# maxipalay/ekf-slam

Measured on AMD Instinct MI355X. Metric: EKF correction steps/sec at N landmarks; pose RMSE vs reference, higher is better.
Workload: dtype f32; 1 GPU; n1024_fp32; n_landmarks=1024, state_dim=2051, filters_per_gpu=1, filters_total=1, markers_per_message=16, association=known, seeds=20240317 + global filter index, survey_messages=640, landmarks_initialised_min=1024, landmarks_initialised_target=1024, inputs=hbm, parallelism=independent filters x1 ranks

## Files before the change

### ekf-slam_amd/csrc/ekf_api.cpp

```cpp
#include <algorithm>
#include <cstdlib>
#include <new>
#include <vector>

#include "ekf_ctx.hpp"
#include "geom.hpp"

using namespace ekfslam;

namespace {

bool valid(ekf_ctx* h, int f) { return h && f >= 0 && f < h->F; }

int load_and_plan(ekf_ctx* h, int assoc_mode, int m_max, const int* counts, const int* ids,
                  const int* actions, const double* rel_xy, const double* odom) {
  Planner& p = h->plan;
  if (int rc = p.load_batch(assoc_mode, m_max, counts, ids, actions, rel_xy, odom)) return rc;
  if (assoc_mode)
    p.unknown(0, h->F, true, true, 0, p.largest(h->F), p.absent(), assoc_route(h));
  else
    p.known(0, h->F, true, p.absent());
  return EKF_OK;
}

// ... 47 lines not shown
  h->ld = (h->n + per_line - 1) / per_line * per_line;
  h->ldk = (h->n + 63) / 64 * 64;
  h->sig_stride = static_cast<size_t>(h->n) * h->ld;
  h->x_stride = static_cast<size_t>((h->n + 15) / 16 * 16);
  h->km_stride = static_cast<size_t>(kMaxKW) * h->ldk;
  h->held.assign(h->F, 0);
  auto fail = [&](int rc) {
    ekf_destroy(h);
    return rc;
  };
  if (hipSetDevice(cfg.device) != hipSuccess) return fail(EKF_E_HIP);
  const char* serial_env = std::getenv("EKF_SERIAL");
  if (serial_env) h->serial = std::atoi(serial_env) != 0;
  if (const char* e = std::getenv("EKF_ASSOC_MSG")) h->assoc_msg = std::atoi(e) != 0;
  {
    const char* e = std::getenv("EKF_RESIDENT");
    h->resident = cfg.dtype == EKF_F64 && h->n <= kResidentMaxN && !(e && std::atoi(e) == 0);
  }
  if (create_streams(h) != EKF_OK ||
      hipEventCreateWithFlags(&h->ev_chain, hipEventDisableTiming) != hipSuccess ||
      hipEventCreateWithFlags(&h->ev_join, hipEventDisableTiming) != hipSuccess ||
      hipEventCreateWithFlags(&h->ev_sig[0], hipEventDisableTiming) != hipSuccess ||
      hipEventCreateWithFlags(&h->ev_sig[1], hipEventDisableTiming) != hipSuccess)
    return fail(EKF_E_HIP);
  if (!serial_env && !h->devsync && h->F > kCuSplitMaxFilters) h->serial = true;
  h->am_route = am_route(h, false);
  h->am_route_j = am_route(h, true);
  if (hipHostMalloc(reinterpret_cast<void**>(&h->fatal_h), 64,
                    hipHostMallocMapped | hipHostMallocCoherent) != hipSuccess)
    return fail(EKF_E_NOMEM);
  *h->fatal_h = 0;
  if (hipHostGetDevicePointer(reinterpret_cast<void**>(&h->fatal_d), h->fatal_h, 0) != hipSuccess)
    return fail(EKF_E_HIP);
  const size_t sig_bytes = h->sig_stride * h->F * h->w;
  for (int p = 0; p < 2; ++p) {
    if (hipMalloc(&h->sig[p], sig_bytes) != hipSuccess) return fail(EKF_E_NOMEM);
    if (hipMalloc(&h->x[p], h->x_stride * h->F * sizeof(double)) != hipSuccess)
      return fail(EKF_E_NOMEM);
  }
  const size_t km_bytes = h->km_stride * h->F * h->w;
  if (hipMalloc(&h->kcat, km_bytes) != hipSuccess) return fail(EKF_E_NOMEM);
  if (hipMalloc(&h->mcat, km_bytes) != hipSuccess) return fail(EKF_E_NOMEM);
  if (hipMalloc(&h->ctl, sizeof(FilterCtl) * h->F) != hipSuccess) return fail(EKF_E_NOMEM);
  if (hipMalloc(&h->rec, 2 * sizeof(ChunkRec) * h->F) != hipSuccess) return fail(EKF_E_NOMEM);
  const char* stage_env = std::getenv("EKF_STAGE");
  const size_t stage_bytes =
      2 * h->F * by_dtype(h, [](auto tag) { return sizeof(StageRec<decltype(tag)>); });
  const bool stage_on = stage_env ? std::atoi(stage_env) != 0
                                  : (h->devsync || h->F <= kCuSplitMaxFilters);
  if (stage_on) {
    if (hipMalloc(&h->stage, stage_bytes) != hipSuccess) return fail(EKF_E_NOMEM);
    if (hipMemset(h->stage, 0, stage_bytes) != hipSuccess) return fail(EKF_E_HIP);
  }
  h->plan.init(h->F, cfg.n_landmarks, h->resident, stage_on);
  const size_t sync_bytes = sizeof(unsigned) * (kSyncChain + static_cast<size_t>(h->F));
  if (hipMalloc(&h->sync, sync_bytes) != hipSuccess) return fail(EKF_E_NOMEM);
  if (hipMemset(h->sync, 0, sync_bytes) != hipSuccess) return fail(EKF_E_HIP);
  h->ddesc_cap = std::max(kDescInit, static_cast<size_t>(h->F) * 4);
  if (hipMalloc(&h->ddesc, sizeof(MsgDesc) * h->ddesc_cap) != hipSuccess) return fail(EKF_E_NOMEM);
  for (int i = 0; i < kRing; ++i)
    if (hipEventCreateWithFlags(&h->ring[i].ev, hipEventDisableTiming) != hipSuccess)
      return fail(EKF_E_HIP);
  if (int rc = reserve_upload(h, h->ddesc_cap)) return fail(rc);
  for (int p = 0; p < 2; ++p) {
    if (hipMemsetAsync(h->sig[p], 0, sig_bytes, h->stream) != hipSuccess) return fail(EKF_E_HIP);
    if (hipMemsetAsync(h->x[p], 0, h->x_stride * h->F * sizeof(double), h->stream) != hipSuccess)
      return fail(EKF_E_HIP);
  }
  if (hipMemsetAsync(h->rec, 0, 2 * sizeof(ChunkRec) * h->F, h->stream) != hipSuccess)
    return fail(EKF_E_HIP);
  if (hipMemsetAsync(h->kcat, 0, km_bytes, h->stream) != hipSuccess ||
      hipMemsetAsync(h->mcat, 0, km_bytes, h->stream) != hipSuccess ||
      hipMemsetAsync(h->ctl, 0, sizeof(FilterCtl) * h->F, h->stream) != hipSuccess)
    return fail(EKF_E_HIP);
  if (init_diag(h, h->sig[0], h->F) || hipStreamSynchronize(h->stream) != hipSuccess)
    return fail(EKF_E_HIP);
  *out = h;
  return EKF_OK;
}

int ekf_destroy(ekf_t h) {
  if (!h) return EKF_E_ARG;
  hipSetDevice(h->cfg.device);
  if (h->bulk) hipStreamSynchronize(h->bulk);
  if (h->stream) hipStreamSynchronize(h->stream);
  for (int p = 0; p < 2; ++p) {
    if (h->sig[p]) hipFree(h->sig[p]);
    if (h->x[p]) hipFree(h->x[p]);
  }
  if (h->kcat) hipFree(h->kcat);
  if (h->mcat) hipFree(h->mcat);
  if (h->ctl) hipFree(h->ctl);
  if (h->rec) hipFree(h->rec);
  if (h->stage) hipFree(h->stage);
  if (h->ddesc) hipFree(h->ddesc);
  for (PlanState* p : h->dstate)
    if (p) hipFree(p);
  if (h->hstate) hipHostFree(h->hstate);
  if (h->odom_d) hipFree(h->odom_d);
  if (h->odom_h) hipHostFree(h->odom_h);
  if (h->ev_odom) hipEventDestroy(h->ev_odom);
  if (h->fatal_h) hipHostFree(h->fatal_h);
  if (h->am.hist) hipFree(h->am.hist);
  if (h->am.cur) hipFree(h->am.cur);
  if (h->am.gran) hipFree(h->am.gran);
  for (int i = 0; i < kRing; ++i) {
// ... 392 lines not shown
```

### ekf-slam_amd/csrc/ekf_chain.hip

```cpp
#include <hip/hip_ext.h>
#include <hip/hip_runtime.h>

#include <cstdint>
#include <type_traits>

#include "ekf_device.hpp"
#include "ekf_launch.hpp"
#include "ekf_math.hpp"
#include "geom.hpp"

namespace ekfslam {

#include "ekf_diag.hpp"
#ifdef EKF_DIAG_STAMPS
__device__ unsigned long long g_stamps[4 * 512];
__device__ double g_blocks[64][kMaxU][kMaxU + 1];
__device__ double g_blockx[64][kMaxU];
}
extern "C" int ekfslam_diag_read_stamps(unsigned long long* out, int n) {
  using ekfslam::g_stamps;
  return hipMemcpyFromSymbol(out, HIP_SYMBOL(g_stamps), sizeof(unsigned long long) * (n < 2048 ? n : 2048)) == hipSuccess ? 0 : -5;
}
extern "C" int ekfslam_diag_read_blocks(double* blocks, double* xs) {
  using namespace ekfslam;
// ... 6 lines not shown
#include "ekf_sync.hpp"

template <bool J>
struct ChainSharedT {
  static constexpr int ZC = J ? kZJ : kZC;
  static constexpr int JM = J ? kMaxJoseph : 1;
  int u[kMaxU];
  int skip[kMaxChunk];
  double alphaU[kMaxU];
  double row0raw[kMaxU];
  double col0raw[kMaxU];
  double xU[1][kMaxU];
  RebuildImage<double> im;
  double Cz[kMaxChunk][4];
  double Dy[kMaxChunk][4];
  double KU[kMaxChunk][kMaxU][2];
  double MU[kMaxChunk][kMaxU][2];
  double Z[kMaxU][ZC + 1];
  double Y[kZC][kMaxU + 1];
  double Zx[kMaxU];
  double nu[kMaxChunk][2];
  double Hs[kMaxChunk][2][5];
  double Sis[kMaxChunk][4];
  double VU[JM][kMaxU][2];
  double Ss[JM][4];
  double Cv[JM][4];
  double Dv[JM][4];
  struct {
    int u[kMaxU];
    int nu, m, first, joseph;
    double a1, a2, s00;
    double xU[kMaxU], Zx[kMaxU];
    double Z[kMaxU + 1][ZC + 1];
    double Y[kZC][kMaxU + 1];
    double K[kMaxU][ZC + 1];
    double M[kZC][kMaxU + 1];
    double r0U[kMaxU], c0U[kMaxU], r0P[kMaxU], c0P[kMaxU];
    double xg[kMaxU];
  } pv;
  double junk[4][64];
  double junk2[64][2];
  double pose[3];
  double xpose[3];
  double npose[3], na1, na2;
  int npose_ci;
  double tmo[3];
  double a1, a2, s00;
  int nu_cnt;
  unsigned status;
  int pub;
  int pdone;
  int any_init;
  int zdone;
};

__device__ __forceinline__ void lds_publish(int* flag, int v) {
  __atomic_signal_fence(__ATOMIC_SEQ_CST);
  __hip_atomic_store(flag, v, __ATOMIC_RELAXED, __HIP_MEMORY_SCOPE_WORKGROUP);
}
__device__ __forceinline__ void lds_wait_ge(const int* flag, int v) {
  while (__builtin_amdgcn_readfirstlane(
             __hip_atomic_load(flag, __ATOMIC_ACQUIRE, __HIP_MEMORY_SCOPE_WORKGROUP)) < v)
    __builtin_amdgcn_s_sleep(1);
}

template <bool J>
using LdsChain = __attribute__((address_space(3))) ChainSharedT<J>;
typedef __attribute__((address_space(3))) const MsgDesc LdsDesc;
typedef __attribute__((address_space(3))) double ldsd;
__device__ __forceinline__ void lds_publish3(__attribute__((address_space(3))) int* flag, int v) {
  __atomic_signal_fence(__ATOMIC_SEQ_CST);
  __hip_atomic_store(flag, v, __ATOMIC_RELAXED, __HIP_MEMORY_SCOPE_WORKGROUP);
}
__device__ __forceinline__ void lds_wait_ge3(const __attribute__((address_space(3))) int* flag,
                                             int v) {
  while (__builtin_amdgcn_readfirstlane(
             __hip_atomic_load(flag, __ATOMIC_ACQUIRE, __HIP_MEMORY_SCOPE_WORKGROUP)) < v)
    __builtin_amdgcn_s_sleep(1);
}

template <bool J>
__device__ __noinline__ void chain_wave0(LdsChain<J>* shp, LdsDesc* dp, int pb, int m, int nu,
                                         double r_noise, unsigned seq) {
  LdsChain<J>& sh = *shp;
  constexpr int JM = ChainSharedT<J>::JM;
  LdsDesc& d = *dp;
  const int lane = threadIdx.x & 63;
  (void)seq;
  const int lr = lane < kMaxU ? lane : kMaxU - 1;
  const int ul = sh.u[lr];
  double pk[5], pm[5];
  double xl = sh.xU[0][lr];
#pragma unroll
  for (int a = 0; a < 5; ++a) {
    const int col = a < 3 ? a : 3 + a - 3;
    pk[a] = sh.im.D[lr][col];
    pm[a] = sh.im.D[col][lr];
  }
  double rn[2], qn[2], kp0 = 0.0, kp1 = 0.0, mp0 = 0.0, mp1 = 0.0, vp0 = 0.0, vp1 = 0.0;
#pragma unroll
  for (int j = 0; j < 2; ++j) {
    const int col = min(5 + j, kMaxU - 1);
    rn[j] = sh.im.D[lr][col];
    qn[j] = sh.im.D[col][lr];
  }
  double lx = 0.0, ly = 0.0, H0[5], H1[5], zhat[2], braw = 0.0;
  bool init = false, bok = true;
// ... 276 lines not shown
  int tid, wv, ln, i16, k4;
};

template <int K>
__device__ __forceinline__ void dot4(const double* a, const double* b, int sb, double (&acc)[4]) {
#pragma unroll
  for (int k = 0; k < K; ++k) acc[k & 3] = fma(a[k], b[k * sb], acc[k & 3]);
}
__device__ __forceinline__ double sum4(const double (&acc)[4]) {
  return (acc[0] + acc[1]) + (acc[2] + acc[3]);
}

template <typename T, bool J>
struct ChainLoads {
  static constexpr int ZC = ChainSharedT<J>::ZC;
  static constexpr int kImPieces = static_cast<int>(sizeof(RebuildImage<T>) / 16);
  static constexpr int kPerIm = (kImPieces + kChainThreads - 1) / kChainThreads;
  static constexpr int kZP = ZC / 2, kZPieces = kMaxU * kZP;
  static constexpr int kPerZ = (kZPieces + kChainThreads - 1) / kChainThreads;
  static constexpr int kYPieces = kZC * kMaxU / 2;
  static constexpr int kPerY = (kYPieces + kChainThreads - 1) / kChainThreads;
  q16 vim[kPerIm], vz[kPerZ], vy[kPerY];
  double r0u, c0u, r0p, c0p, x2;
  double x0, x1, pa1, pa2, tq;
  int pflags;
};

template <typename T, bool J>
__device__ __forceinline__ void load_prev_record(ChainLoads<T, J>& L, __amdgpu_buffer_rsrc_t rr,
                                                 int tid) {
  using CL = ChainLoads<T, J>;
  constexpr unsigned oZ = offsetof(ChunkRec, Z), oY = offsetof(ChunkRec, Y);
  const int tc = tid < kMaxU ? tid : 0;
#pragma unroll
  for (int i = 0; i < CL::kPerZ; ++i) {
    const int p = tid + i * kChainThreads, pz = p < CL::kZPieces ? p : 0;
    L.vz[i] = ld_q16(rr, oZ + 8u * ((pz / CL::kZP) * kZJ + 2 * (pz % CL::kZP)));
  }
#pragma unroll
  for (int i = 0; i < CL::kPerY; ++i) {
    const int p = tid + i * kChainThreads;
    L.vy[i] = ld_q16(rr, oY + 16u * (p < CL::kYPieces ? p : 0));
  }
  L.x0 = ld_f64(rr, offsetof(ChunkRec, xU) + 8u * tc, 0);
  L.x1 = ld_f64(rr, offsetof(ChunkRec, Zx) + 8u * tc, 0);
  L.pflags = static_cast<int>(__builtin_amdgcn_raw_buffer_load_b32(rr, offsetof(ChunkRec, flags), 0, 0));
  L.pa1 = ld_f64(rr, offsetof(ChunkRec, a1), 0);
  L.pa2 = ld_f64(rr, offsetof(ChunkRec, a2), 0);
}

template <typename T, bool J>
__device__ __forceinline__ void issue_early_loads(ChainLoads<T, J>& L, const StageRec<T>* sg,
                                                  const ChunkRec* rp, FilterCtl* ctl, int tid,
                                                  bool early) {
  using CL = ChainLoads<T, J>;
  const int tc = tid < kMaxU ? tid : 0;
  const auto rs = buf_rsrc(sg, early ? static_cast<unsigned>(sizeof(StageRec<T>)) : 0u);
  constexpr unsigned oIm = offsetof(StageRec<T>, im);
#pragma unroll
  for (int i = 0; i < CL::kPerIm; ++i) {
    const int p = tid + i * kChainThreads;
    L.vim[i] = ld_q16(rs, oIm + 16u * (p < CL::kImPieces ? p : 0));
  }
  load_prev_record(L, buf_rsrc(rp, early ? static_cast<unsigned>(sizeof(ChunkRec)) : 0u), tid);
  L.r0u = ld_f64(rs, offsetof(StageRec<T>, r0u) + 8u * tc, 0);
  L.c0u = ld_f64(rs, offsetof(StageRec<T>, c0u) + 8u * tc, 0);
  L.r0p = ld_f64(rs, offsetof(StageRec<T>, r0p) + 8u * tc, 0);
  L.c0p = ld_f64(rs, offsetof(StageRec<T>, c0p) + 8u * tc, 0);
  L.x2 = ld_f64(rs, offsetof(StageRec<T>, xg) + 8u * tc, 0);
  L.tq = ctl->tmo[tid < 3 ? tid : 0];
}

__device__ __forceinline__ bool bad_id(int id, int N) { return id < 0 || id >= N; }
__device__ __forceinline__ int column_of_id(int id, int N, int tid) {
  return (bad_id(id, N) ? 3 : 3 + 2 * id) + ((tid - 3) & 1);
}

template <bool J>
__device__ __forceinline__ void build_index_sets(ChainSharedT<J>& sh, const MsgDesc& d, int N, int aj,
                                                 bool look, int tid) {
  const int m = d.m;
  if (tid < kMaxU) {
    int u = tid < 3 ? tid : 0;
    if (tid >= 3 && tid < 3 + 2 * m) {
      const int c = (tid - 3) >> 1, idd = d.ids[c];
      const int id = idd >= 0 ? idd : aj;
      const bool bad = bad_id(id, N);
      u = column_of_id(id, N, tid);
      if (((tid - 3) & 1) == 0) {
        sh.skip[c] = bad ? 1 : 0;
        if (bad && idd >= 0) atomicOr(&sh.status, EKF_FLAG_RANGE_D);
      }
    }
    sh.u[tid] = u;
  }
  if (tid == 0) sh.nu_cnt = 3 + 2 * m;
  if (look && tid < kMaxU) {
    const int pm = d.prev_m;
    int u = 0;
    if (tid < 3) {
      u = tid;
    } else if (tid < 3 + 2 * pm) {
      u = column_of_id(d.prev_ids[(tid - 3) >> 1], N, tid);
    }
    sh.pv.u[tid] = u;
    if (tid == 0) {
      sh.pv.nu = 3 + 2 * pm;
      sh.pv.m = pm;
    }
  }
}

template <typename T, bool J>
__device__ __forceinline__ void land_rebuild_operands(ChainSharedT<J>& sh, ChainLoads<T, J>& L,
                                                      const T* Sp, const double* xp, int ld,
                                                      const ChunkRec* rp, FilterCtl* ctl, int tid,
                                                      int nu, int np, bool early) {
  using CL = ChainLoads<T, J>;
  constexpr int ZC = CL::ZC;
  static_assert(sizeof(sh.im) == 2 * sizeof(RebuildImage<float>) && alignof(decltype(sh.im)) >= 16 &&
                    (kZC * kMaxU) % 2 == 0 && ZC % 2 == 0,
                "the staged image and the record's Z / Y are copied in 16-byte pieces");
  const int tc = tid < kMaxU ? tid : 0;
  if (!early) {
    load_prev_record(L, buf_rsrc(rp, static_cast<unsigned>(sizeof(ChunkRec))), tid);
    T vd[kRebPer], vr[kRebPer], vc[kRebPer];
#pragma unroll
    for (int i = 0; i < kRebPer; ++i) {
      const int e = tid + i * kChainThreads;
      const int a = min(e / kRebW, kMaxU - 1), b = min(e % kRebW, kMaxU - 1);
      const size_t ua = static_cast<size_t>(sh.u[a]) * ld, pa = static_cast<size_t>(sh.pv.u[b]);
      vd[i] = Sp[ua + sh.u[b]];
      vr[i] = Sp[ua + pa];
      vc[i] = Sp[pa * ld + sh.u[a]];
    }
    const int uu = sh.u[tc], pu = sh.pv.u[tc];
    L.r0u = static_cast<double>(Sp[uu]);
    L.c0u = static_cast<double>(Sp[static_cast<size_t>(uu) * ld]);
    L.r0p = static_cast<double>(Sp[pu]);
    L.c0p = static_cast<double>(Sp[static_cast<size_t>(pu) * ld]);
    L.x2 = xp[uu];
    L.tq = ctl->tmo[tid < 3 ? tid : 0];
    store_raw_image<T>(sh, vd, vr, vc, tid, nu, np);
  } else {
    d2m* const im = reinterpret_cast<d2m*>(&sh.im);
#pragma unroll
    for (int i = 0; i < CL::kPerIm; ++i) {
      const int p = tid + i * kChainThreads;
      if (p < CL::kImPieces) {
        if constexpr (sizeof(T) == 8) {
          im[p] = __builtin_bit_cast(d2m, L.vim[i]);
        } else {
          const f4v w = __builtin_bit_cast(f4v, L.vim[i]);
          im[2 * p] = d2m{static_cast<double>(w.x), static_cast<double>(w.y)};
          im[2 * p + 1] = d2m{static_cast<double>(w.z), static_cast<double>(w.w)};
        }
      }
    }
  }
#pragma unroll
  for (int i = 0; i < CL::kPerZ; ++i) {
    const int p = tid + i * kChainThreads;
    const d2m w = __builtin_bit_cast(d2m, L.vz[i]);
    if (p < CL::kZPieces) {
      double* z = &sh.pv.Z[p / CL::kZP][2 * (p % CL::kZP)];
      z[0] = w.x;
      z[1] = w.y;
    }
  }
#pragma unroll
  for (int i = 0; i < CL::kPerY; ++i) {
    const int p = tid + i * kChainThreads, e0 = 2 * p, e1 = 2 * p + 1;
    const d2m w = __builtin_bit_cast(d2m, L.vy[i]);
    if (p < CL::kYPieces) {
      sh.pv.Y[e0 / kMaxU][e0 % kMaxU] = w.x;
      sh.pv.Y[e1 / kMaxU][e1 % kMaxU] = w.y;
    }
  }
  if (tid < ZC) sh.pv.Z[kMaxU][tid] = 0.0;
  if (tid < kZC) sh.pv.Y[tid][kMaxU] = 0.0;
  if (tid < kMaxU) {
    sh.pv.r0U[tid] = L.r0u;
    sh.pv.c0U[tid] = L.c0u;
    sh.pv.r0P[tid] = L.r0p;
    sh.pv.c0P[tid] = L.c0p;
    sh.pv.xU[tid] = L.x0;
    sh.pv.Zx[tid] = L.x1;
    sh.pv.xg[tid] = L.x2;
  }
  if (tid == 0) {
    sh.pv.first = (L.pflags & kFirst) != 0;
    sh.pv.joseph = (L.pflags & kJoseph) != 0;
    sh.pv.a1 = L.pa1;
    sh.pv.a2 = L.pa2;
  }
  if (tid < 3) sh.tmo[tid] = L.tq;
}

template <bool J>
__device__ __forceinline__ double prev_x_at_U(ChainSharedT<J>& sh, int ln, int np) {
  const int l = ln < kMaxU ? ln : kMaxU - 1;
  const int u = sh.u[l];
  int pos = -1;
#pragma unroll
  for (int k = kMaxU - 1; k >= 0; --k) pos = (k < np && sh.pv.u[k] == u) ? k : pos;
  double bacc[4] = {0.0, 0.0, 0.0, 0.0};
  dot4<kMaxU>(&sh.im.R[l][0], &sh.pv.Zx[0], 1, bacc);
  const double r = sum4(bacc);
  return pos >= 0 ? sh.pv.xU[pos] : sh.pv.xg[l] + r;
}

template <bool J>
__device__ __forceinline__ void km_band_dot(ChainSharedT<J>& sh, bool bk, int brow, int bcol,
                                            double (&bacc)[4]) {
  const double* ra = bk ? &sh.im.R[min(brow, kMaxU - 1)][0] : &sh.pv.Y[brow][0];
  const double* cb = bk ? &sh.pv.Z[0][bcol] : &sh.im.C[0][min(bcol, kMaxU)];
  const int sc = bk ? ChainSharedT<J>::ZC + 1 : kMaxU + 1;
  dot4<kMaxU + 1>(ra, cb, sc, bacc);
}

template <bool W3>
__device__ __forceinline__ void rebuild_km_simple(ChainSharedT<false>& sh, const ChainLane& L, int nu,
                                                  int np) {
  const int tid = L.tid, wv = L.wv, ln = L.ln, i16 = L.i16, k4 = L.k4;
  double av[2][9], bv[2][9];
#pragma unroll
  for (int q = 0; q < 2; ++q) {
    const int tt = wv + 4 * q;
    const bool kt = tt < 4;
    const int ti = (kt ? tt : tt - 4) >> 1, tj = (kt ? tt : tt - 4) & 1;
    const double* pa = kt ? &sh.im.R[16 * ti + i16][0] : &sh.pv.Y[16 * ti + i16][0];
    const double* pb = kt ? &sh.pv.Z[0][16 * tj + i16] : &sh.im.C[0][16 * tj + i16];
    const int sb = kt ? kZC + 1 : kMaxU + 1;
#pragma unroll
    for (int s0 = 0; s0 < 9; ++s0) {
      av[q][s0] = pa[4 * s0 + k4];
      bv[q][s0] = pb[(4 * s0 + k4) * sb];
    }
  }
  double bacc[4] = {0.0, 0.0, 0.0, 0.0};
  int brow = 0, bcol = 0;
  bool bk = false;
  double xres = 0.0;
  if (!W3) {
    if (tid < 96) {
      bk = true;
      brow = 32 + (tid >> 5);
      bcol = tid & 31;
    } else {
// ... 126 lines not shown
    for (int tj = 0; tj < 3; ++tj) {
      const int bc = min(16 * tj + i16, kMaxU - 1);
#pragma unroll
      for (int r = 0; r < 4; ++r) acc[tj][r] = P[min(16 * wv + k4 + 4 * r, kMaxU - 1)][bc];
    }
#pragma unroll
    for (int h = 0; h < 2; ++h) {
      double bv[3][8];
#pragma unroll
      for (int tj = 0; tj < 3; ++tj) {
        const int bc = min(16 * tj + i16, kMaxU - 1);
#pragma unroll
        for (int s0 = 0; s0 < 8; ++s0)
          bv[tj][s0] = h == 0 ? sh.pv.M[4 * s0 + k4][bc] : (pj ? sh.pv.K[bc][4 * s0 + k4] : 0.0);
      }
#pragma unroll
      for (int s0 = 0; s0 < 8; ++s0)
#pragma unroll
        for (int tj = 0; tj < 3; ++tj) acc[tj] = mfma_f64(av[8 * h + s0], bv[tj][s0], acc[tj]);
    }
#pragma unroll
    for (int tj = 0; tj < 3; ++tj) {
      const int col = 16 * tj + i16;
#pragma unroll
      for (int r = 0; r < 4; ++r) {
        const int row = 16 * wv + k4 + 4 * r;
        if (row < nu && col < nu) P[row][col] = acc[tj][r];
      }
    }
  }
}

template <bool J>
__device__ __forceinline__ void pick_predicted_pose(ChainSharedT<J>& sh, const MsgDesc& d, int ci) {
  if (sh.npose_ci == ci) {
    sh.pose[0] = sh.npose[0];
    sh.pose[1] = sh.npose[1];
    sh.pose[2] = sh.npose[2];
    sh.a1 = sh.na1;
    sh.a2 = sh.na2;
  } else {
    double a1, a2;
    const double xp[3] = {sh.pv.xU[0], sh.pv.xU[1], sh.pv.xU[2]};
    predicted_pose(sh.tmo, d, xp, sh.pose, &a1, &a2);
    sh.a1 = a1;
    sh.a2 = a2;
  }
}

template <typename T, bool J>
__device__ __forceinline__ void rebuild_block(ChainSharedT<J>& sh, const MsgDesc& d,
                                              ChainLoads<T, J>& loads, const T* Sp, const double* xp,
                                              int ld, const ChunkRec* rp, FilterCtl* ctl,
                                              const ChainLane& L, int nu, bool early, double q, int ci,
                                              unsigned seq) {
  (void)seq;
  const int np = sh.pv.nu;
  land_rebuild_operands(sh, loads, Sp, xp, ld, rp, ctl, L.tid, nu, np, early);
  __syncthreads();
  EKF_STAMP(21);
  predict_prev(sh, L.tid, nu, np, q);
  __syncthreads();

  EKF_STAMP(3);
  EKF_STAMP(4);
  if constexpr (!J)
    L.wv == 3 ? rebuild_km_simple<true>(sh, L, nu, np) : rebuild_km_simple<false>(sh, L, nu, np);
  else
    L.wv == 3 ? rebuild_km_joseph<true>(sh, L, nu, np) : rebuild_km_joseph<false>(sh, L, nu, np);
  EKF_STAMP(7);
  __syncthreads();
  EKF_STAMP(5);
  if constexpr (!J)
    rebuild_p_simple(sh, L, nu);
  else
    rebuild_p_joseph(sh, L, nu);
  EKF_STAMPT(10, 64);
  EKF_STAMPT(11, 128);
  EKF_STAMPT(13, 192);
  if (L.wv == 2 && L.ln == 0) {
    pick_predicted_pose(sh, d, ci);
    EKF_STAMPT(8, 128);
  }
  EKF_STAMPT(9, 192);
}

template <typename T, bool J>
__device__ __forceinline__ void gather_block(ChainSharedT<J>& sh, const MsgDesc& d, const T* S,
                                             const double* xin, int ld, FilterCtl* ctl, int tid,
                                             int nu) {
  auto& P = sh.im.D;
  double vd[kRebPer];
#pragma unroll
  for (int i = 0; i < kRebPer; ++i) {
    const int e = tid + i * kChainThreads;
    const int a = min(e / kRebW, kMaxU - 1), b = min(e % kRebW, kMaxU - 1);
    vd[i] = static_cast<double>(S[static_cast<size_t>(sh.u[a]) * ld + sh.u[b]]);
  }
  const double xv = xin[sh.u[tid < nu ? tid : 0]];
  const double xq = xin[tid < 3 ? tid : 0];
  const double tq = ctl->tmo[tid < 3 ? tid : 0];
#pragma unroll
  for (int i = 0; i < kRebPer; ++i) {
    const int e = tid + i * kChainThreads;
    const int a = e / kRebW, b = e % kRebW;
    if (a < nu && b < nu) P[a][b] = vd[i];
  }
  if (tid < nu) sh.xU[0][tid] = xv;
  if (tid < 3) {
    sh.xpose[tid] = xq;
    sh.tmo[tid] = tq;
  }
// ... 434 lines not shown
        st_wt(&rec->Y[2 * c][lane], in ? y0 : 0.0);
        st_wt(&rec->Y[2 * c + 1][lane], in ? y1 : 0.0);
      }
    }
    EKF_STAMPT(360 + c, 128);
  }
}

template <bool J>
__device__ __forceinline__ void write_pend_patch(ChainSharedT<J>& sh, ChunkRec* rec, int m, int nu,
                                                 int tid, bool joseph) {
  constexpr int JM = ChainSharedT<J>::JM;
  auto& P = sh.im.D;
  const int c = max(m - 1, 0);
  for (int e = tid; e < kMaxU * kMaxU; e += blockDim.x) {
    const int a = e / kMaxU, b = e - a * kMaxU;
    double v = P[a][b];
    if (m > 0)
      v = rank2_sub(v, sh.KU[c][a][0], sh.KU[c][a][1], sh.MU[c][b][0], sh.MU[c][b][1]);
    if (m > 0 && joseph) {
      const int cj = min(c, JM - 1);
      v = rank2_sub(v, sh.VU[cj][a][0], sh.VU[cj][a][1], sh.KU[c][b][0], sh.KU[c][b][1]);
    }
    if (a < nu && b < nu) st_wt(&rec->Pend[a][b], v);
  }
}

template <bool J>
__device__ __forceinline__ void write_record(ChainSharedT<J>& sh, const MsgDesc& d, ChunkRec* rec,
                                             FilterCtl* ctl, int m, int nu, int tid, bool pend) {
  const double* xfin = sh.xU[0];
  if (tid == 0 && sh.status) atomicOr(&ctl->status, sh.status);
  if (tid < kMaxU) {
    const double zx = sh.Zx[tid];
    const bool in = tid < nu;
    st_wt(&rec->Zx[tid], zx);
    st_wt(&rec->u[tid], sh.u[tid]);
    st_wt(&rec->alphaU[tid], in ? sh.alphaU[tid] : 0.0);
    st_wt(&rec->row0raw[tid], in ? sh.row0raw[tid] : 0.0);
    st_wt(&rec->col0raw[tid], in ? sh.col0raw[tid] : 0.0);
    st_wt(&rec->xU[tid], in ? xfin[tid] : 0.0);
  }
  if (tid == 0) {
    st_wt(&rec->m, m);
    st_wt(&rec->nu, nu);
    st_wt(&rec->flags, d.flags | (pend ? kPendValid : 0));
    st_wt(&rec->a1, sh.a1);
    st_wt(&rec->a2, sh.a2);
    st_wt(&rec->s00, sh.s00);
  }
}

template <typename T, bool J>
__global__ __launch_bounds__(kChainThreads) void k_chain(PassArgs<T> A, int nchunks) {
  __shared__ ChainSharedT<J> sh;
  __shared__ MsgDesc sdesc[2];
  static_assert(sizeof(MsgDesc) % 16 == 0, "MsgDesc copied as uint4");
  const int fy = blockIdx.y;
  const int f = A.f0 + fy;
  const int tid = threadIdx.x;
  const int ld = A.ld;
  FilterCtl* ctl = A.ctl + f;
  for (int e = tid; e < static_cast<int>(sizeof(sh) / 8); e += blockDim.x)
    reinterpret_cast<double*>(&sh)[e] = 0.0;
  __syncthreads();
  if (tid == 0) sh.npose_ci = -1;
  bool pre = false;
  unsigned pending = 0;
  for (int ci = 0; ci < nchunks; ++ci) {
    if (!pre) {
      const MsgDesc& gd = A.desc[static_cast<size_t>(ci) * A.desc_stride + fy];
      if (ci == 0 && A.need_plan && tid == 0 && !epoch_wait_acquire(A.sync + kSyncPlan, A.need_plan))
        flag_timeout(&ctl->status, A.fatal);
      __syncthreads();
      if (threadIdx.x < sizeof(MsgDesc) / 16)
        reinterpret_cast<uint4*>(&sdesc[ci & 1])[threadIdx.x] =
            reinterpret_cast<const uint4*>(&gd)[threadIdx.x];
      __syncthreads();
    }
    pre = false;
    const MsgDesc& d = sdesc[ci & 1];
    auto& P = sh.im.D;
    (void)P;
    const bool active = (d.flags & kActive) != 0;
    const bool look = (d.flags & kLook) != 0 && !A.gather;
    if (pending) {
      drain_stores();
      __syncthreads();
      if (tid == 0) epoch_store(A.sync + kSyncChain + f, pending);
      pending = 0;
    }
    if (!active) continue;
    const unsigned seq = A.seq + static_cast<unsigned>(ci);
    const unsigned need = look ? (seq >= 2 ? seq - 1 : 0u) : seq;
    const int cA = tid >= 3 && tid < 3 + 2 * d.m ? (tid - 3) >> 1 : 0;
    const int aj = ctl->assoc_j[min(max(d.assoc_slot + cA, 0), kMaxAssoc - 1)];
    if (A.polls && need && tid == 0 && !(A.first_ready && need <= A.seq) &&
        !epoch_wait_acquire(A.sync + kSyncSigma, need))
      flag_timeout(&ctl->status, A.fatal);
    EKF_STAMP(305);
    if (tid == 0) sh.status = 0;
    __syncthreads();
    EKF_STAMP(0);
    const T* S = A.sig[d.parity] + f * A.sig_stride;
    const double* xin = A.x[d.parity] + f * A.x_stride;
    const int m = d.m;
    const bool first = (d.flags & kFirst) != 0;
    const bool joseph = J && (d.flags & kJoseph) != 0;
    const ChunkRec* rp = A.rec + static_cast<size_t>(d.parity ^ 1) * A.rec_stride + f;

    const bool early = look && (d.flags & kStageIn);
    ChainLoads<T, J> loads;
    issue_early_loads(loads, A.stage + static_cast<size_t>(d.parity) * A.rec_stride + f, rp, ctl,
                      tid, early);
    EKF_STAMP(14);

    build_index_sets(sh, d, A.N, aj, look, tid);
    lds_barrier();
    EKF_STAMP(1);
    const int nu = sh.nu_cnt;
    const ChainLane L = {tid, tid >> 6, tid & 63, tid & 15, (tid & 63) >> 4};

    if (look)
      rebuild_block(sh, d, loads, A.sig[d.parity ^ 1] + f * A.sig_stride,
                    A.x[d.parity ^ 1] + f * A.x_stride, ld, rp, ctl, L, nu, early, A.q, ci, seq);
    else
      gather_block(sh, d, S, xin, ld, ctl, tid, nu);
    EKF_STAMP(6);

    __syncthreads();
    fold_predict(sh, tid, nu, first, A.q);
    __syncthreads();
    EKF_STAMP(2);
    EKF_DUMP_BLOCK(seq);
    EKF_STAMP(18);

    if (tid == 0) {
      sh.pub = 0;
      sh.pdone = 0;
      sh.zdone = 0;
      sh.any_init = 0;
    }
    if (pending) drain_stores();
    __syncthreads();
    if (pending) {
      if (tid == 0) epoch_store(A.sync + kSyncChain + f, pending);
      pending = 0;
    }
    EKF_STAMP(19);
    const bool pre_next = ci + 1 < nchunks;
    ChunkRec* const rec = A.rec + static_cast<size_t>(d.parity) * A.rec_stride + f;
    if (L.wv == 0)
      chain_wave0<J>((LdsChain<J>*)(&sh), (LdsDesc*)(&d), 0, m, nu, A.r, seq);
    else if (L.wv == 3)
      chain_wave3(sh, d, A, ctl, fy, m, nu, L.ln, ci, nchunks, seq);
    else if (L.wv == 1)
      chain_wave1(sh, rec, m, nu, L.ln, seq);
    else
      chain_wave2(sh, rec, m, nu, L.ln, joseph, seq);
    __syncthreads();

    const bool pend = sizeof(T) == 4 && (sh.any_init || (d.flags & kNoInit));
    if (pend) write_pend_patch(sh, rec, m, nu, tid, joseph);
    __syncthreads();
    EKF_STAMP(12);

    if (L.wv != 3) {
      if (pre_next && tid >= 128 && tid < 128 + static_cast<int>(sizeof(MsgDesc) / 16))
        reinterpret_cast<uint4*>(&sdesc[(ci + 1) & 1])[tid - 128] =
            reinterpret_cast<const uint4*>(
                &A.desc[static_cast<size_t>(ci + 1) * A.desc_stride + fy])[tid - 128];
      write_record(sh, d, rec, ctl, m, nu, tid, pend);
      EKF_STAMP(16);
    }
    pending = seq + 1u;
    pre = pre_next;
    __syncthreads();
    EKF_STAMP(40);
    EKF_STAMPV(307, __builtin_amdgcn_s_memrealtime());
  }
  if (pending) {
    drain_stores();
    __syncthreads();
    if (tid == 0) epoch_store(A.sync + kSyncChain + f, pending);
  }
}
template <typename T>
hipError_t launch_chain(const PassArgs<T>& a, int nf, int nchunks, hipStream_t s, hipEvent_t e0,
                        hipEvent_t e1) {
  launch(a.joseph ? k_chain<T, true> : k_chain<T, false>, dim3(1, nf), dim3(kChainThreads), s, e0,
         e1, a, nchunks);
  return hipGetLastError();
}
template hipError_t launch_chain<double>(const PassArgs<double>&, int, int, hipStream_t, hipEvent_t,
                                         hipEvent_t);
template hipError_t launch_chain<float>(const PassArgs<float>&, int, int, hipStream_t, hipEvent_t,
                                        hipEvent_t);

}
```

### ekf-slam_amd/csrc/ekf_ctx.hpp

```cpp
#pragma once
#include <hip/hip_ext.h>
#include <hip/hip_runtime.h>

#include <vector>

#include "ekf.h"
#include "ekf_device.hpp"
#include "ekf_launch.hpp"
#include "ekf_plan.hpp"

namespace ekfslam {

constexpr int kRing = 16;

struct StageSlot {
  MsgDesc* p = nullptr;
  size_t cap = 0;
  hipEvent_t ev = nullptr;
  bool used = false;
};

struct ProfEvents {
  std::vector<hipEvent_t> start, stop;
};

enum ProfSlot : int {
  kProfSigma = 0,
  kProfChain = 1,
  kProfAssoc = 2,
  kProfFactors = 3,
  kProfResident = 4,
  kProfSlots = 5,
};

}

static_assert(EKF_RESIDENT_MAX_N == ekfslam::kResidentMaxN, "ekf.h and ekf_launch.hpp agree");

struct ekf_ctx {
  ekf_config cfg{};
  int n = 0, ld = 0, ldk = 0, F = 0;
  size_t w = 8;
  hipStream_t stream = nullptr;
  hipStream_t bulk = nullptr;
  bool serial = false;
  bool resident = false;
  bool defer = false;
  bool assoc_msg = true;
  bool main_dirty = false;
  bool main_unordered = false;
  bool epoch_owed = false;
  ekfslam::AmArgs am{};
  int am_route = 0;
  int am_route_j = 0;
  int am_group = 1;
  int am_group_j = 1;
  int bulk_cus_per_xcd = 0;
  int main_cus_per_xcd = 0;
  unsigned* fatal_h = nullptr;
  unsigned* fatal_d = nullptr;
  hipEvent_t ev_chain = nullptr;
  hipEvent_t ev_join = nullptr;
  bool devsync = false;
  unsigned* sync = nullptr;
  hipEvent_t ev_sig[2] = {nullptr, nullptr};
  long long seq = 0;
  void* sig[2] = {nullptr, nullptr};
  double* x[2] = {nullptr, nullptr};
  void* kcat = nullptr;
  void* mcat = nullptr;
  ekfslam::FilterCtl* ctl = nullptr;
  ekfslam::ChunkRec* rec = nullptr;
  void* stage = nullptr;
  ekfslam::MsgDesc* ddesc = nullptr;
  size_t sig_stride = 0, x_stride = 0, km_stride = 0;
  ekfslam::PlanState* dstate[2] = {nullptr, nullptr};
  ekfslam::PlanState* hstate = nullptr;
  int dstate_cur = 0;
  bool dev_plan = false;
  hipStream_t plan_stream = nullptr;
  unsigned plan_total = 0;
  unsigned need_plan = 0;
  double* odom_d = nullptr;
  double* odom_h = nullptr;
  size_t odom_cap = 0;
  hipEvent_t ev_odom = nullptr;
  ekfslam::Planner plan;
  std::vector<unsigned> held;
  size_t ddesc_cap = 0;
  ekfslam::StageSlot ring[ekfslam::kRing];
  size_t ring_cap = 0;
  int ring_next = 0;
  bool prof = false;
  ekfslam::ProfEvents pe[ekfslam::kProfSlots];
  std::vector<hipEvent_t> pool;
  long long prof_launches[ekfslam::kProfSlots] = {0, 0, 0, 0, 0};
  long long prof_chunks = 0;
  double prof_ms[ekfslam::kProfSlots] = {0, 0, 0, 0, 0};
};

#define HIPCHK(expr)                       \
  do {                                     \
    if ((expr) != hipSuccess) return EKF_E_HIP; \
  } while (0)

namespace ekfslam {

template <typename Fn>
auto by_dtype(const ekf_ctx* h, Fn fn) {
  return h->cfg.dtype == EKF_F32 ? fn(float{}) : fn(double{});
}

constexpr int kCuSplitMaxFilters = 32;
constexpr size_t kDescInit = 256;
int create_streams(ekf_ctx* h);
int am_route(ekf_ctx* h, bool joseph);
// ... 27 lines not shown
```

### ekf-slam_amd/csrc/ekf_launch.hpp

```cpp
#pragma once
#include <hip/hip_ext.h>
#include <hip/hip_runtime.h>

#include <cstddef>

#include "ekf_device.hpp"

namespace ekfslam {

template <typename T>
struct PassArgs {
  T* sig[2];
  size_t sig_stride;
  double* x[2];
  size_t x_stride;
  T* kcat;
  T* mcat;
  size_t km_stride;
  int ldk;
  FilterCtl* ctl;
  ChunkRec* rec;
  size_t rec_stride;
  StageRec<T>* stage;
  unsigned* sync;
  unsigned* fatal;
  unsigned seq;
  unsigned need_sigma;
  unsigned need_plan;
  unsigned pub_sigma;
  int first_ready;
  int polls;
  int gather;
  const MsgDesc* desc;
  int desc_stride;
  int n, ld, N, f0;
  double q, r, gate;
  int joseph;
};

template <typename K, typename... Args>
void launch(K kernel, dim3 grid, dim3 block, hipStream_t s, hipEvent_t e0, hipEvent_t e1,
            Args... args) {
  if (e0 && e1)
    hipExtLaunchKernelGGL(kernel, grid, block, 0, s, e0, e1, 0, args...);
  else
    hipLaunchKernelGGL(kernel, grid, block, 0, s, args...);
}

template <typename T>
hipError_t launch_chain(const PassArgs<T>& a, int n_filters, int nchunks, hipStream_t s,
                        hipEvent_t e0 = nullptr, hipEvent_t e1 = nullptr);

template <typename T>
hipError_t launch_factors(const PassArgs<T>& a, int n_filters, hipStream_t s,
                      hipEvent_t e0 = nullptr, hipEvent_t e1 = nullptr);

template <typename T>
hipError_t launch_sigma_pass(const PassArgs<T>& a, int n_filters, bool publish, bool stage, hipStream_t s,
                      hipEvent_t e0 = nullptr, hipEvent_t e1 = nullptr);

template <typename T>
hipError_t launch_assoc(const PassArgs<T>& a, int n_filters, hipStream_t s,
                      hipEvent_t e0 = nullptr, hipEvent_t e1 = nullptr);

struct AmArgs {
  AmHist* hist;
  AmCur* cur;
  unsigned long long* gran;
  size_t hist_stride, cur_stride, gran_stride;
  int G;
  int xcd;
  unsigned spin;
  int drop;
  double prior;
};
int assoc_msg_blocks_per_cu(bool f32, bool joseph);
template <typename T>
hipError_t launch_assoc_msg(const PassArgs<T>& a, const AmArgs& b, int n_filters, hipStream_t s,
                            hipEvent_t e0 = nullptr, hipEvent_t e1 = nullptr);

template <typename T>
hipError_t launch_posterior(const PassArgs<T>& a, int n_filters, hipStream_t s);

constexpr int kResidentMaxN = 128;
hipError_t launch_resident(const PassArgs<double>& a, const PlanEntry* plan, int nplan, int flo,
// ... 40 lines not shown
```

### ekf-slam_amd/csrc/ekf_sched.cpp

```cpp
#include <algorithm>
#include <climits>
#include <cstdlib>
#include <cstring>

#include "ekf_ctx.hpp"
#include "ekf_internal.hpp"

namespace ekfslam {

namespace {

template <typename T>
PassArgs<T> args(ekf_ctx* h, const MsgDesc* desc, int f0) {
  PassArgs<T> a{};
  a.sig[0] = static_cast<T*>(h->sig[0]);
  a.sig[1] = static_cast<T*>(h->sig[1]);
  a.sig_stride = h->sig_stride;
  a.x[0] = h->x[0];
  a.x[1] = h->x[1];
  a.x_stride = h->x_stride;
  a.kcat = static_cast<T*>(h->kcat);
  a.mcat = static_cast<T*>(h->mcat);
  a.km_stride = h->km_stride;
  a.ldk = h->ldk;
  a.ctl = h->ctl;
  a.rec = h->rec;
  a.rec_stride = static_cast<size_t>(h->F);
  a.stage = static_cast<StageRec<T>*>(h->stage);
  a.sync = h->sync;
  a.fatal = h->fatal_d;
  a.desc = desc;
  a.n = h->n;
  a.ld = h->ld;
  a.N = h->cfg.n_landmarks;
  a.f0 = f0;
  a.q = h->cfg.q_noise;
  a.r = h->cfg.r_noise;
  a.gate = h->cfg.mah_gate;
  a.joseph = h->plan.joseph() ? 1 : 0;
  return a;
}

hipEvent_t pool_get(ekf_ctx* h) {
  if (!h->pool.empty()) {
    hipEvent_t e = h->pool.back();
    h->pool.pop_back();
    return e;
  }
  hipEvent_t e = nullptr;
  if (hipEventCreate(&e) != hipSuccess) return nullptr;
  return e;
}

template <typename Fn>
int timed(ekf_ctx* h, ProfSlot kind, Fn fn) {
  hipEvent_t a = nullptr, b = nullptr;
  if (h->prof) {
    a = pool_get(h);
    b = pool_get(h);
  }
  const hipError_t e = fn(a && b ? a : nullptr, a && b ? b : nullptr);
  if (h->prof && a && b) {
    h->pe[kind].start.push_back(a);
    h->pe[kind].stop.push_back(b);
  }
  return e == hipSuccess ? EKF_OK : EKF_E_HIP;
}

int join_bulk(ekf_ctx* h) {
  if (hipEventRecord(h->ev_join, h->bulk) != hipSuccess ||
      hipStreamWaitEvent(h->stream, h->ev_join, 0) != hipSuccess)
    return EKF_E_HIP;
  return EKF_OK;
}

int fork_bulk(ekf_ctx* h) {
  HIPCHK(hipEventRecord(h->ev_chain, h->stream));
  HIPCHK(hipStreamWaitEvent(h->bulk, h->ev_chain, 0));
  return EKF_OK;
}

int fork_bulk_clean(ekf_ctx* h) {
  if (fork_bulk(h)) return EKF_E_HIP;
// ... 618 lines not shown
```

Baseline: 537,400 corrections/s.

## Overlap chunk boundary work: early next-descriptor fetch, epoch poll, record from LDS

For fp32 non-Joseph chains, one wave now fetches the next message descriptor during the current chunk's wave work. Wave 0 then polls the sigma epoch for the next chunk early, so the boundary wait moves off the critical path. The previous chunk's Z/Y/xU record is copied from LDS instead of reloaded from global memory. The chain-epoch publish is deferred into the rebuild barrier. Both behaviours sit behind an EKF_BOUNDARY mask that defaults on. The cost is more intra-workgroup LDS flag synchronisation and extra ordering subtlety.

```diff
diff --git a/ekf-slam_amd/csrc/ekf_api.cpp b/ekf-slam_amd/csrc/ekf_api.cpp
--- a/ekf-slam_amd/csrc/ekf_api.cpp
+++ b/ekf-slam_amd/csrc/ekf_api.cpp
@@ -123,6 +123,7 @@
     if (hipMalloc(&h->stage, stage_bytes) != hipSuccess) return fail(EKF_E_NOMEM);
     if (hipMemset(h->stage, 0, stage_bytes) != hipSuccess) return fail(EKF_E_HIP);
   }
+  if (const char* e = std::getenv("EKF_BOUNDARY")) h->boundary = std::atoi(e) & 3;
   h->plan.init(h->F, cfg.n_landmarks, h->resident, stage_on);
   const size_t sync_bytes = sizeof(unsigned) * (kSyncChain + static_cast<size_t>(h->F));
   if (hipMalloc(&h->sync, sync_bytes) != hipSuccess) return fail(EKF_E_NOMEM);
diff --git a/ekf-slam_amd/csrc/ekf_chain.hip b/ekf-slam_amd/csrc/ekf_chain.hip
--- a/ekf-slam_amd/csrc/ekf_chain.hip
+++ b/ekf-slam_amd/csrc/ekf_chain.hip
@@ -82,7 +82,12 @@
   int pdone;
   int any_init;
   int zdone;
+  int nd_ci;
 };
+
+constexpr int kBndEpoch = 1, kBndRecord = 2;
+template <typename T, bool J>
+constexpr bool kBoundaryForm = sizeof(T) == 4 && !J;
 
 __device__ __forceinline__ void lds_publish(int* flag, int v) {
   __atomic_signal_fence(__ATOMIC_SEQ_CST);
@@ -465,7 +470,7 @@
 template <typename T, bool J>
 __device__ __forceinline__ void issue_early_loads(ChainLoads<T, J>& L, const StageRec<T>* sg,
                                                   const ChunkRec* rp, FilterCtl* ctl, int tid,
-                                                  bool early) {
+                                                  bool early, bool early_rec) {
   using CL = ChainLoads<T, J>;
   const int tc = tid < kMaxU ? tid : 0;
   const auto rs = buf_rsrc(sg, early ? static_cast<unsigned>(sizeof(StageRec<T>)) : 0u);
@@ -475,13 +480,19 @@
     const int p = tid + i * kChainThreads;
     L.vim[i] = ld_q16(rs, oIm + 16u * (p < CL::kImPieces ? p : 0));
   }
-  load_prev_record(L, buf_rsrc(rp, early ? static_cast<unsigned>(sizeof(ChunkRec)) : 0u), tid);
+  load_prev_record(L, buf_rsrc(rp, early_rec ? static_cast<unsigned>(sizeof(ChunkRec)) : 0u), tid);
   L.r0u = ld_f64(rs, offsetof(StageRec<T>, r0u) + 8u * tc, 0);
   L.c0u = ld_f64(rs, offsetof(StageRec<T>, c0u) + 8u * tc, 0);
   L.r0p = ld_f64(rs, offsetof(StageRec<T>, r0p) + 8u * tc, 0);
   L.c0p = ld_f64(rs, offsetof(StageRec<T>, c0p) + 8u * tc, 0);
   L.x2 = ld_f64(rs, offsetof(StageRec<T>, xg) + 8u * tc, 0);
-  L.tq = ctl->tmo[tid < 3 ? tid : 0];
+  if constexpr (kBoundaryForm<T, J>) {
+    const bool tmo_lds = early && !early_rec;
+    L.tq = ld_f64(buf_rsrc(ctl->tmo, tmo_lds ? 0u : static_cast<unsigned>(sizeof(ctl->tmo))),
+                  8u * (tid < 3 ? tid : 0), 0);
+  } else {
+    L.tq = ctl->tmo[tid < 3 ? tid : 0];
+  }
 }
 
 __device__ __forceinline__ bool bad_id(int id, int N) { return id < 0 || id >= N; }
@@ -524,17 +535,49 @@
   }
 }
 
+__device__ __forceinline__ void record_from_lds(ChainSharedT<false>& sh, const MsgDesc& pd,
+                                                int tid) {
+  const int m = pd.m, nu = 3 + 2 * m;
+  constexpr int kPer = (kMaxU * kZC + kChainThreads - 1) / kChainThreads;
+  double vz[kPer], vy[kPer];
+#pragma unroll
+  for (int i = 0; i < kPer; ++i) {
+    const int e = min(tid + i * kChainThreads, kMaxU * kZC - 1);
+    vz[i] = sh.Z[e / kZC][e % kZC];
+    vy[i] = sh.Y[e / kMaxU][e % kMaxU];
+  }
+#pragma unroll
+  for (int i = 0; i < kPer; ++i) {
+    const int e = min(tid + i * kChainThreads, kMaxU * kZC - 1);
+    sh.pv.Z[e / kZC][e % kZC] = e % kZC < 2 * m ? vz[i] : 0.0;
+    sh.pv.Y[e / kMaxU][e % kMaxU] = e / kMaxU < 2 * m ? vy[i] : 0.0;
+  }
+  if (tid < kMaxU) {
+    sh.pv.xU[tid] = tid < nu ? sh.xU[0][tid] : 0.0;
+    sh.pv.Zx[tid] = sh.Zx[tid];
+  }
+  if (tid == 0) {
+    sh.pv.first = (pd.flags & kFirst) != 0;
+    sh.pv.joseph = (pd.flags & kJoseph) != 0;
+    sh.pv.a1 = sh.a1;
+    sh.pv.a2 = sh.a2;
+  }
+}
+__device__ __forceinline__ void record_from_lds(ChainSharedT<true>&, const MsgDesc&, int) {}
+
 template <typename T, bool J>
 __device__ __forceinline__ void land_rebuild_operands(ChainSharedT<J>& sh, ChainLoads<T, J>& L,
                                                       const T* Sp, const double* xp, int ld,
                                                       const ChunkRec* rp, FilterCtl* ctl, int tid,
-                                                      int nu, int np, bool early) {
+                                                      int nu, int np, bool early, bool lrec,
+                                                      const MsgDesc& pd) {
   using CL = ChainLoads<T, J>;
   constexpr int ZC = CL::ZC;
   static_assert(sizeof(sh.im) == 2 * sizeof(RebuildImage<float>) && alignof(decltype(sh.im)) >= 16 &&
                     (kZC * kMaxU) % 2 == 0 && ZC % 2 == 0,
                 "the staged image and the record's Z / Y are copied in 16-byte pieces");
   const int tc = tid < kMaxU ? tid : 0;
+  if (lrec) record_from_lds(sh, pd, tid);
   if (!early) {
     load_prev_record(L, buf_rsrc(rp, static_cast<unsigned>(sizeof(ChunkRec))), tid);
     T vd[kRebPer], vr[kRebPer], vc[kRebPer];
@@ -571,23 +614,25 @@
       }
     }
   }
-#pragma unroll
-  for (int i = 0; i < CL::kPerZ; ++i) {
-    const int p = tid + i * kChainThreads;
-    const d2m w = __builtin_bit_cast(d2m, L.vz[i]);
-    if (p < CL::kZPieces) {
-      double* z = &sh.pv.Z[p / CL::kZP][2 * (p % CL::kZP)];
-      z[0] = w.x;
-      z[1] = w.y;
-    }
-  }
-#pragma unroll
-  for (int i = 0; i < CL::kPerY; ++i) {
-    const int p = tid + i * kChainThreads, e0 = 2 * p, e1 = 2 * p + 1;
-    const d2m w = __builtin_bit_cast(d2m, L.vy[i]);
-    if (p < CL::kYPieces) {
-      sh.pv.Y[e0 / kMaxU][e0 % kMaxU] = w.x;
-      sh.pv.Y[e1 / kMaxU][e1 % kMaxU] = w.y;
+  if (!lrec) {
+#pragma unroll
+    for (int i = 0; i < CL::kPerZ; ++i) {
+      const int p = tid + i * kChainThreads;
+      const d2m w = __builtin_bit_cast(d2m, L.vz[i]);
+      if (p < CL::kZPieces) {
+        double* z = &sh.pv.Z[p / CL::kZP][2 * (p % CL::kZP)];
+        z[0] = w.x;
+        z[1] = w.y;
+      }
+    }
+#pragma unroll
+    for (int i = 0; i < CL::kPerY; ++i) {
+      const int p = tid + i * kChainThreads, e0 = 2 * p, e1 = 2 * p + 1;
+      const d2m w = __builtin_bit_cast(d2m, L.vy[i]);
+      if (p < CL::kYPieces) {
+        sh.pv.Y[e0 / kMaxU][e0 % kMaxU] = w.x;
+        sh.pv.Y[e1 / kMaxU][e1 % kMaxU] = w.y;
+      }
     }
   }
   if (tid < ZC) sh.pv.Z[kMaxU][tid] = 0.0;
@@ -597,17 +642,21 @@
     sh.pv.c0U[tid] = L.c0u;
     sh.pv.r0P[tid] = L.r0p;
     sh.pv.c0P[tid] = L.c0p;
-    sh.pv.xU[tid] = L.x0;
-    sh.pv.Zx[tid] = L.x1;
     sh.pv.xg[tid] = L.x2;
   }
-  if (tid == 0) {
-    sh.pv.first = (L.pflags & kFirst) != 0;
-    sh.pv.joseph = (L.pflags & kJoseph) != 0;
-    sh.pv.a1 = L.pa1;
-    sh.pv.a2 = L.pa2;
-  }
-  if (tid < 3) sh.tmo[tid] = L.tq;
+  if (!lrec) {
+    if (tid < kMaxU) {
+      sh.pv.xU[tid] = L.x0;
+      sh.pv.Zx[tid] = L.x1;
+    }
+    if (tid == 0) {
+      sh.pv.first = (L.pflags & kFirst) != 0;
+      sh.pv.joseph = (L.pflags & kJoseph) != 0;
+      sh.pv.a1 = L.pa1;
+      sh.pv.a2 = L.pa2;
+    }
+    if (tid < 3) sh.tmo[tid] = L.tq;
+  }
 }
 
 template <bool J>
@@ -840,12 +889,21 @@
 __device__ __forceinline__ void rebuild_block(ChainSharedT<J>& sh, const MsgDesc& d,
                                               ChainLoads<T, J>& loads, const T* Sp, const double* xp,
                                               int ld, const ChunkRec* rp, FilterCtl* ctl,
-                                              const ChainLane& L, int nu, bool early, double q, int ci,
-                                              unsigned seq) {
+                                              const ChainLane& L, int nu, bool early, bool lrec,
+                                              const MsgDesc& pd, unsigned* chain_epoch,
+                                              unsigned& pending, double q, int ci, unsigned seq) {
   (void)seq;
   const int np = sh.pv.nu;
-  land_rebuild_operands(sh, loads, Sp, xp, ld, rp, ctl, L.tid, nu, np, early);
+  land_rebuild_operands(sh, loads, Sp, xp, ld, rp, ctl, L.tid, nu, np, early, lrec, pd);
+  if constexpr (kBoundaryForm<T, J>)
+    if (pending) drain_stores();
   __syncthreads();
+  if constexpr (kBoundaryForm<T, J>) {
+    if (pending) {
+      if (L.tid == 0) epoch_store(chain_epoch, pending);
+      pending = 0;
+    }
+  }
   EKF_STAMP(21);
   predict_prev(sh, L.tid, nu, np, q);
   __syncthreads();
@@ -1386,6 +1444,15 @@
 }
 
 template <typename T, bool J>
+__device__ __forceinline__ int next_boundary(int boundary, int gather, const MsgDesc& d,
+                                             const MsgDesc& nd) {
+  constexpr int kNeed = kActive | kLook | kStageIn;
+  const bool ok = kBoundaryForm<T, J> && !gather && (d.flags & kActive) && (nd.flags & kNeed) == kNeed &&
+                  nd.parity == (d.parity ^ 1) && nd.prev_m == d.m;
+  return ok ? boundary & (kBndEpoch | kBndRecord) : 0;
+}
+
+template <typename T, bool J>
 __global__ __launch_bounds__(kChainThreads) void k_chain(PassArgs<T> A, int nchunks) {
   __shared__ ChainSharedT<J> sh;
   __shared__ MsgDesc sdesc[2];
@@ -1398,7 +1465,10 @@
   for (int e = tid; e < static_cast<int>(sizeof(sh) / 8); e += blockDim.x)
     reinterpret_cast<double*>(&sh)[e] = 0.0;
   __syncthreads();
-  if (tid == 0) sh.npose_ci = -1;
+  if (tid == 0) {
+    sh.npose_ci = -1;
+    sh.nd_ci = -1;
+  }
   bool pre = false;
   unsigned pending = 0;
   for (int ci = 0; ci < nchunks; ++ci) {
@@ -1418,7 +1488,10 @@
     (void)P;
     const bool active = (d.flags & kActive) != 0;
     const bool look = (d.flags & kLook) != 0 && !A.gather;
-    if (pending) {
+    const MsgDesc& pd = sdesc[(ci & 1) ^ 1];
+    const int bnd = ci > 0 ? next_boundary<T, J>(A.boundary, A.gather, pd, d) : 0;
+    const bool polled = (bnd & kBndEpoch) != 0, lrec = (bnd & kBndRecord) != 0;
+    if (pending && !(kBoundaryForm<T, J> && lrec)) {
       drain_stores();
       __syncthreads();
       if (tid == 0) epoch_store(A.sync + kSyncChain + f, pending);
@@ -1429,7 +1502,7 @@
     const unsigned need = look ? (seq >= 2 ? seq - 1 : 0u) : seq;
     const int cA = tid >= 3 && tid < 3 + 2 * d.m ? (tid - 3) >> 1 : 0;
     const int aj = ctl->assoc_j[min(max(d.assoc_slot + cA, 0), kMaxAssoc - 1)];
-    if (A.polls && need && tid == 0 && !(A.first_ready && need <= A.seq) &&
+    if (A.polls && need && tid == 0 && !polled && !(A.first_ready && need <= A.seq) &&
         !epoch_wait_acquire(A.sync + kSyncSigma, need))
       flag_timeout(&ctl->status, A.fatal);
     EKF_STAMP(305);
@@ -1446,7 +1519,7 @@
     const bool early = look && (d.flags & kStageIn);
     ChainLoads<T, J> loads;
     issue_early_loads(loads, A.stage + static_cast<size_t>(d.parity) * A.rec_stride + f, rp, ctl,
-                      tid, early);
+                      tid, early, early && !lrec);
     EKF_STAMP(14);
 
     build_index_sets(sh, d, A.N, aj, look, tid);
@@ -1457,7 +1530,8 @@
 
     if (look)
       rebuild_block(sh, d, loads, A.sig[d.parity ^ 1] + f * A.sig_stride,
-                    A.x[d.parity ^ 1] + f * A.x_stride, ld, rp, ctl, L, nu, early, A.q, ci, seq);
+                    A.x[d.parity ^ 1] + f * A.x_stride, ld, rp, ctl, L, nu, early, lrec, pd,
+                    A.sync + kSyncChain + f, pending, A.q, ci, seq);
     else
       gather_block(sh, d, S, xin, ld, ctl, tid, nu);
     EKF_STAMP(6);
@@ -1475,23 +1549,40 @@
       sh.zdone = 0;
       sh.any_init = 0;
     }
-    if (pending) drain_stores();
     __syncthreads();
-    if (pending) {
-      if (tid == 0) epoch_store(A.sync + kSyncChain + f, pending);
-      pending = 0;
-    }
     EKF_STAMP(19);
     const bool pre_next = ci + 1 < nchunks;
+    const bool early_desc = kBoundaryForm<T, J> && (A.boundary & kBndEpoch) != 0;
     ChunkRec* const rec = A.rec + static_cast<size_t>(d.parity) * A.rec_stride + f;
-    if (L.wv == 0)
+    if (L.wv == 0) {
       chain_wave0<J>((LdsChain<J>*)(&sh), (LdsDesc*)(&d), 0, m, nu, A.r, seq);
-    else if (L.wv == 3)
+      EKF_STAMP(22);
+      if constexpr (kBoundaryForm<T, J>) {
+        if (pre_next && early_desc) {
+          lds_wait_ge(&sh.nd_ci, ci + 1);
+          __atomic_signal_fence(__ATOMIC_SEQ_CST);
+          EKF_STAMP(23);
+          const unsigned nneed = seq + 1u >= 2u ? seq : 0u;
+          if ((next_boundary<T, J>(A.boundary, A.gather, d, sdesc[(ci + 1) & 1]) & kBndEpoch) &&
+              A.polls && nneed && L.ln == 0 && !(A.first_ready && nneed <= A.seq) &&
+              !epoch_wait_acquire(A.sync + kSyncSigma, nneed))
+            flag_timeout(&ctl->status, A.fatal);
+          EKF_STAMP(24);
+        }
+      }
+    } else if (L.wv == 3) {
       chain_wave3(sh, d, A, ctl, fy, m, nu, L.ln, ci, nchunks, seq);
-    else if (L.wv == 1)
+    } else if (L.wv == 1) {
       chain_wave1(sh, rec, m, nu, L.ln, seq);
-    else
+    } else {
+      if (pre_next && early_desc) {
+        if (L.ln < static_cast<int>(sizeof(MsgDesc) / 16))
+          reinterpret_cast<uint4*>(&sdesc[(ci + 1) & 1])[L.ln] = reinterpret_cast<const uint4*>(
+              &A.desc[static_cast<size_t>(ci + 1) * A.desc_stride + fy])[L.ln];
+        lds_publish(&sh.nd_ci, ci + 1);
+      }
       chain_wave2(sh, rec, m, nu, L.ln, joseph, seq);
+    }
     __syncthreads();
 
     const bool pend = sizeof(T) == 4 && (sh.any_init || (d.flags & kNoInit));
@@ -1500,7 +1591,8 @@
     EKF_STAMP(12);
 
     if (L.wv != 3) {
-      if (pre_next && tid >= 128 && tid < 128 + static_cast<int>(sizeof(MsgDesc) / 16))
+      if (pre_next && !early_desc && tid >= 128 &&
+          tid < 128 + static_cast<int>(sizeof(MsgDesc) / 16))
         reinterpret_cast<uint4*>(&sdesc[(ci + 1) & 1])[tid - 128] =
             reinterpret_cast<const uint4*>(
                 &A.desc[static_cast<size_t>(ci + 1) * A.desc_stride + fy])[tid - 128];
diff --git a/ekf-slam_amd/csrc/ekf_ctx.hpp b/ekf-slam_amd/csrc/ekf_ctx.hpp
--- a/ekf-slam_amd/csrc/ekf_ctx.hpp
+++ b/ekf-slam_amd/csrc/ekf_ctx.hpp
@@ -62,6 +62,7 @@
   hipEvent_t ev_chain = nullptr;
   hipEvent_t ev_join = nullptr;
   bool devsync = false;
+  int boundary = 3;
   unsigned* sync = nullptr;
   hipEvent_t ev_sig[2] = {nullptr, nullptr};
   long long seq = 0;
diff --git a/ekf-slam_amd/csrc/ekf_launch.hpp b/ekf-slam_amd/csrc/ekf_launch.hpp
--- a/ekf-slam_amd/csrc/ekf_launch.hpp
+++ b/ekf-slam_amd/csrc/ekf_launch.hpp
@@ -31,6 +31,7 @@
   int first_ready;
   int polls;
   int gather;
+  int boundary;
   const MsgDesc* desc;
   int desc_stride;
   int n, ld, N, f0;
diff --git a/ekf-slam_amd/csrc/ekf_sched.cpp b/ekf-slam_amd/csrc/ekf_sched.cpp
--- a/ekf-slam_amd/csrc/ekf_sched.cpp
+++ b/ekf-slam_amd/csrc/ekf_sched.cpp
@@ -29,6 +29,7 @@
   a.stage = static_cast<StageRec<T>*>(h->stage);
   a.sync = h->sync;
   a.fatal = h->fatal_d;
+  a.boundary = h->boundary;
   a.desc = desc;
   a.n = h->n;
   a.ld = h->ld;
```

Result: slower. 531,300 corrections/s (-1.1%).
